# ddlee-cn/LeRF-PyTorch

Measured on AMD Instinct MI355X. Metric: Mpix/s LeRF-G x2 SR (2K->4K), higher is better.
Workload: dtype i32+f32 (u8 io); 1 GPU; LeRF-G LUT x2 SR, 1920x1080->3840x2160 RGB uint8, S=2, max_sigma=10 (BASELINE configs[1]); input=noise, mode=frames, parallelism=independent frames per GPU, no data-path collective, ranks_reported_by_rccl=1, channels=3, library=lerf-pytorch_amd/liblerf_hip.so

## Files before the change

### lerf-pytorch_amd/csrc/lerf_fused_impl.h

```cpp
#include <string.h>
#include <atomic>
#include <type_traits>

#include "lerf_kernels.h"
#include "lerf_stage3.h"
#include "lerf_warp_px.h"

namespace lerf {
namespace LERF_FUSED_NS {

#ifndef LERF_FUSED_NT
#define LERF_FUSED_NT 1024
#endif
constexpr int NT = LERF_FUSED_NT;
constexpr int NW = NT / 64;
constexpr int CH = LERF_FUSED_CH;
static_assert(CH == 1 || CH == 3 || CH == 4, "192 pixel-channels per tile row");
#ifndef LERF_FUSED_TH
#define LERF_FUSED_TH 64
#endif
constexpr int TH = LERF_FUSED_TH, TW = 192 / CH;
constexpr int R1 = 3, R2 = 3;
constexpr int MAXM = 4;
constexpr int LUT_PAD = 83584;
// ... 201 lines not shown
    __device__ __forceinline__ uint32_t ld32(int n) const { return n >= 3 ? lds_ld32<ALL>(a(n)) : lds_ld32<0>(a(n)); }
    __device__ __forceinline__ int ldi8(int n) const { return n >= 3 ? lds_ldi8<ALL>(a(n)) : lds_ldi8<0>(a(n)); }
};

template <int STRIDE_SCALE>
__device__ __forceinline__ Walk<STRIDE_SCALE> simplex_walk(unsigned ka, int basea, uint32_t rb, uint32_t rc, uint32_t rd,
                                                           unsigned sb, unsigned sc, unsigned sd) {
    Walk<STRIDE_SCALE> W;
    const unsigned kb = key_of(rb, sb), kc = key_of(rc, sc), kd = key_of(rd, sd);
    const unsigned t = __umul24(__umul24(msb_of(rb), (unsigned)kL) + msb_of(rc), (unsigned)kL) + msb_of(rd);
    W.i0 = basea + (int)(t * STRIDE_SCALE);
    const unsigned m = umax3(ka, kb, kc), e = umed3(ka, kb, kc), n = umin3(ka, kb, kc);
    const unsigned s0 = m > kd ? m : kd;
    const unsigned s1 = umed3(m, e, kd);
    const unsigned s2 = umed3(e, n, kd);
    const unsigned s3 = n < kd ? n : kd;
    W.i1 = W.i0 + (int)(s0 & 0xFFFFu);
    W.i2 = W.i1 + (int)(s1 & 0xFFFFu);
    W.i3m = W.i0 - (int)(s3 & 0xFFFFu);
    W.f0 = s0 >> 16; W.f1 = s1 >> 16; W.f2 = s2 >> 16; W.f3 = s3 >> 16;
    W.k0 = s0; W.k1 = s1; W.k2 = s2; W.k3 = s3;
    return W;
}

template <int BYTES>
struct Stage16 {
    static constexpr int n = (BYTES + 15) >> 4;
    static constexpr int FULL = n / NT;
    static constexpr int TAIL = n - FULL * NT;
    uint4 r[FULL];
    uint4 rt;
    __device__ __forceinline__ void load(const uint8_t* __restrict__ src, int tid) {
        const uint4* s = reinterpret_cast<const uint4*>(src);
#pragma unroll
        for (int i = 0; i < FULL; ++i) r[i] = s[tid + i * NT];
        rt = make_uint4(0, 0, 0, 0);
        if (TAIL > 0 && tid < TAIL) rt = s[tid + FULL * NT];
    }
    __device__ __forceinline__ void store(uint8_t* dst, int tid) const {
        uint4* d = reinterpret_cast<uint4*>(dst);
#pragma unroll
        for (int i = 0; i < FULL; ++i) d[tid + i * NT] = r[i];
        if (TAIL > 0 && tid < TAIL) d[tid + FULL * NT] = rt;
    }
};

template <int BYTES>
__device__ __forceinline__ void copy16(uint8_t* dst, const uint8_t* __restrict__ src, int tid) {
    Stage16<BYTES> st;
    st.load(src, tid);
    st.store(dst, tid);
}

template <int SP>
__host__ __device__ constexpr int min_tile_offset(char mode, int rot0, int nrot, int rstep) {
    int m = 0;
    for (int i = 0; i < nrot; ++i) {
        const Off3 o = tile_offsets<SP>(mode, rot0 + i * rstep);
        for (int k = 0; k < 3; ++k) m = o.o[k] < m ? o.o[k] : m;
    }
    return m;
}
template <int SP>
__host__ __device__ constexpr int block3_offset(int i) {
    const int dy = i < 3 ? -1 : (i < 5 ? 0 : 1);
    const int dx = i < 3 ? i - 1 : (i < 5 ? (i == 3 ? -1 : 1) : i - 6);
    return dy * SP + dx * CH;
}
template <int SP>
__host__ __device__ constexpr int block3_index(int off) {
    for (int i = 0; i < 8; ++i)
        if (block3_offset<SP>(i) == off) return i;
    return 0;
}
template <int SP, char MODE, int ROT, int MINO>
__device__ __forceinline__ void load_rotation(uint32_t base, uint32_t& rb, uint32_t& rc, uint32_t& rd) {
    constexpr Off3 o = tile_offsets<SP>(MODE, ROT);
    rb = lds_pixel_hi_off<o.o[0] - MINO>(base);
    rc = lds_pixel_hi_off<o.o[1] - MINO>(base);
    rd = lds_pixel_hi_off<o.o[2] - MINO>(base);
}

template <int NROT>
__device__ __forceinline__ int byte_walks(uint32_t lut_a, uint32_t ra, const uint32_t (&rb)[4], const uint32_t (&rc)[4],
                                          const uint32_t (&rd)[4]) {
    const unsigned sa = kStrideA, sb = kStrideB, sc = kStrideC, sd = kStrideD;
    const unsigned ka = key_of(ra, sa);
    const int basea = (int)(__umul24(msb_of(ra), kStrideA) + lut_a);
    Walk<1> W[NROT];
    int e[NROT][5];
#ifndef LERF_S1_SPLIT
#define LERF_S1_SPLIT 1
#endif
#if LERF_S1_SPLIT > 0
#pragma unroll
    for (int h = 0; h < NROT; h += LERF_S1_SPLIT) {
#pragma unroll
        for (int i = h; i < h + LERF_S1_SPLIT; ++i) W[i] = simplex_walk<1>(ka, basea, rb[i], rc[i], rd[i], sb, sc, sd);
#pragma unroll
        for (int i = h; i < h + LERF_S1_SPLIT; ++i)
#pragma unroll
            for (int n = 0; n < 5; ++n) e[i][n] = W[i].ldi8(n);
        __builtin_amdgcn_sched_barrier(0);
    }
#else
#pragma unroll
    for (int i = 0; i < NROT; ++i) W[i] = simplex_walk<1>(ka, basea, rb[i], rc[i], rd[i], sb, sc, sd);
#pragma unroll
    for (int i = 0; i < NROT; ++i)
#pragma unroll
        for (int n = 0; n < 5; ++n) e[i][n] = W[i].ldi8(n);
    __builtin_amdgcn_sched_barrier(0);
#endif
    int acc = 0, sum0 = 0;
#pragma unroll
    for (int i = 0; i < NROT; ++i) {
        sum0 += e[i][0];
#ifndef LERF_S1_MUL24
        acc = mad_i16_keyhi(e[i][1] - e[i][0], W[i].k0, acc);
        acc = mad_i16_keyhi(e[i][2] - e[i][1], W[i].k1, acc);
        acc = mad_i16_keyhi(e[i][3] - e[i][2], W[i].k2, acc);
        acc = mad_i16_keyhi(e[i][4] - e[i][3], W[i].k3, acc);
#else
        acc += __mul24((int)W[i].f0, e[i][1] - e[i][0]);
        acc += __mul24((int)W[i].f1, e[i][2] - e[i][1]);
        acc += __mul24((int)W[i].f2, e[i][3] - e[i][2]);
        acc += __mul24((int)W[i].f3, e[i][4] - e[i][3]);
#endif
    }
    return acc + kQ * sum0;
}


template <int SP, char MODE, int ROT0, int NROT, int RSTEP>
__device__ __forceinline__ int byte_lookups(uint32_t lut_a, uint32_t center) {
    static_assert(NROT == 2 || NROT == 4, "rotation pairs or all four");
    constexpr int MINO = min_tile_offset<SP>(MODE, ROT0, NROT, RSTEP);
    const uint32_t base = center + (uint32_t)MINO;
    uint32_t ra = lds_pixel_hi_off<-MINO>(base);
    uint32_t rb[4], rc[4], rd[4];
    if constexpr (MODE == 's' && NROT == 4 && ROT0 == 0 && RSTEP == 1) {
        uint32_t nb[8];
        nb[0] = lds_pixel_hi_off<block3_offset<SP>(0) - MINO>(base); nb[1] = lds_pixel_hi_off<block3_offset<SP>(1) - MINO>(base);
        nb[2] = lds_pixel_hi_off<block3_offset<SP>(2) - MINO>(base); nb[3] = lds_pixel_hi_off<block3_offset<SP>(3) - MINO>(base);
        nb[4] = lds_pixel_hi_off<block3_offset<SP>(4) - MINO>(base); nb[5] = lds_pixel_hi_off<block3_offset<SP>(5) - MINO>(base);
        nb[6] = lds_pixel_hi_off<block3_offset<SP>(6) - MINO>(base); nb[7] = lds_pixel_hi_off<block3_offset<SP>(7) - MINO>(base);
        asm volatile("s_waitcnt lgkmcnt(0)"
                     : "+v"(ra), "+v"(nb[0]), "+v"(nb[1]), "+v"(nb[2]), "+v"(nb[3]), "+v"(nb[4]), "+v"(nb[5]), "+v"(nb[6]), "+v"(nb[7]));
#pragma unroll
        for (int r = 0; r < 4; ++r) {
            const Off3 o = tile_offsets<SP>('s', r);
            rb[r] = nb[block3_index<SP>(o.o[0])];
            rc[r] = nb[block3_index<SP>(o.o[1])];
            rd[r] = nb[block3_index<SP>(o.o[2])];
        }
    } else {
    load_rotation<SP, MODE, ROT0, MINO>(base, rb[0], rc[0], rd[0]);
    load_rotation<SP, MODE, ROT0 + RSTEP, MINO>(base, rb[1], rc[1], rd[1]);
    if constexpr (NROT == 4) {
        load_rotation<SP, MODE, ROT0 + 2 * RSTEP, MINO>(base, rb[2], rc[2], rd[2]);
        load_rotation<SP, MODE, ROT0 + 3 * RSTEP, MINO>(base, rb[3], rc[3], rd[3]);
        asm volatile("s_waitcnt lgkmcnt(0)"
                     : "+v"(ra), "+v"(rb[0]), "+v"(rc[0]), "+v"(rd[0]), "+v"(rb[1]), "+v"(rc[1]), "+v"(rd[1]), "+v"(rb[2]),
                       "+v"(rc[2]), "+v"(rd[2]), "+v"(rb[3]), "+v"(rc[3]), "+v"(rd[3]));
    } else {
        asm volatile("s_waitcnt lgkmcnt(0)" : "+v"(ra), "+v"(rb[0]), "+v"(rc[0]), "+v"(rd[0]), "+v"(rb[1]), "+v"(rc[1]), "+v"(rd[1]));
    }
    }
    return byte_walks<NROT>(lut_a, ra, rb, rc, rd);
}

template <int NROT>
__device__ __forceinline__ int byte_lookups_rt(uint32_t lut_a, uint32_t center, const int* __restrict__ o) {
    static_assert(NROT == 2 || NROT == 4, "rotation pairs or all four");
    uint32_t ra = lds_pixel_hi(center);
    uint32_t rb[4], rc[4], rd[4];
#pragma unroll
    for (int i = 0; i < NROT; ++i) {
        rb[i] = lds_pixel_hi(center + (uint32_t)o[3 * i]);
        rc[i] = lds_pixel_hi(center + (uint32_t)o[3 * i + 1]);
        rd[i] = lds_pixel_hi(center + (uint32_t)o[3 * i + 2]);
    }
    if constexpr (NROT == 4)
        asm volatile("s_waitcnt lgkmcnt(0)"
                     : "+v"(ra), "+v"(rb[0]), "+v"(rc[0]), "+v"(rd[0]), "+v"(rb[1]), "+v"(rc[1]), "+v"(rd[1]), "+v"(rb[2]),
                       "+v"(rc[2]), "+v"(rd[2]), "+v"(rb[3]), "+v"(rc[3]), "+v"(rd[3]));
    else
        asm volatile("s_waitcnt lgkmcnt(0)" : "+v"(ra), "+v"(rb[0]), "+v"(rc[0]), "+v"(rd[0]), "+v"(rb[1]), "+v"(rc[1]), "+v"(rd[1]));
    return byte_walks<NROT>(lut_a, ra, rb, rc, rd);
}

template <int DPc, int SP>
__device__ __forceinline__ int center_addr(int p, int y0g, int x0g, int sy0g, int sx0g, int H, int W, bool* inside) {
    int ry = p / DPc;
    int r3 = p - ry * DPc;
    if (H < 0) {
        if (inside) *inside = true;
        return (ry + (y0g - sy0g)) * SP + r3 + (x0g - sx0g) * CH;
    }
    int rx = r3 / CH;
    int c = r3 - rx * CH;
    int gy = y0g + ry, gx = x0g + rx;
    int cy = clampi(gy, 0, H - 1), cx = clampi(gx, 0, W - 1);
    if (inside) *inside = (cy == gy) && (cx == gx);
    return (cy - sy0g) * SP + (cx - sx0g) * CH + c;
}

template <int NDST, int DPc, int SP, char MODE, int ROT0, int NROT, int RSTEP, int PHASE>
__device__ __forceinline__ void byte_position(uint32_t lut_a, uint32_t center, int16_t* acc16, uint8_t* dst8, int p, int div, int bias) {
    int v = byte_lookups<SP, MODE, ROT0, NROT, RSTEP>(lut_a, center);
    if (PHASE != 0) v += (int)acc16[p];
    if (PHASE == 2)
        dst8[p] = (uint8_t)rne_div_clip255_fast(v + bias * div, div);
// ... 8 lines not shown
    if (H < 0) {
        constexpr int FULL = NDST / NT, TAIL = NDST - FULL * NT;
        const uint32_t org = src_a + (uint32_t)((y0g - sy0g) * SP + (x0g - sx0g) * CH);
#pragma unroll 1
        for (int k = 0; k < FULL; ++k) {
            const int p = tid + k * NT;
            const int ry = p / DPc;
            byte_position<NDST, DPc, SP, MODE, ROT0, NROT, RSTEP, PHASE>(lut_a, org + (uint32_t)(ry * (SP - DPc) + p), acc16, dst8, p, div, bias);
        }
        if (TAIL > 0 && tid < TAIL) {
            const int p = tid + FULL * NT;
            const int ry = p / DPc;
            byte_position<NDST, DPc, SP, MODE, ROT0, NROT, RSTEP, PHASE>(lut_a, org + (uint32_t)(ry * (SP - DPc) + p), acc16, dst8, p, div, bias);
        }
        return;
    }
    for (int p = tid; p < NDST; p += NT) {
        bool in = true;
        int a = center_addr<DPc, SP>(p, y0g, x0g, sy0g, sx0g, H, W, SKIP_OUTSIDE ? &in : nullptr);
        if (SKIP_OUTSIDE && !in) continue;
        byte_position<NDST, DPc, SP, MODE, ROT0, NROT, RSTEP, PHASE>(lut_a, src_a + (uint32_t)a, acc16, dst8, p, div, bias);
    }
}

struct DyDx { int dy[3], dx[3]; };
__host__ __device__ constexpr DyDx pattern_dydx(char mode, int rot) {
    int dy[4] = {0, 0, 0, 0}, dx[4] = {0, 0, 0, 0};
    switch (mode) {
        case 's': dy[1] = 0; dx[1] = 1; dy[2] = 1; dx[2] = 0; dy[3] = 1; dx[3] = 1; break;
        case 'd': dy[1] = 0; dx[1] = 2; dy[2] = 2; dx[2] = 0; dy[3] = 2; dx[3] = 2; break;
        case 'y': dy[1] = 1; dx[1] = 1; dy[2] = 1; dx[2] = 2; dy[3] = 2; dx[3] = 1; break;
        case 'c': dy[1] = 0; dx[1] = 1; dy[2] = 0; dx[2] = 2; dy[3] = 0; dx[3] = 3; break;
        default:  dy[1] = 1; dx[1] = 1; dy[2] = 2; dx[2] = 2; dy[3] = 3; dx[3] = 3; break;
    }
    DyDx r{};
    for (int k = 1; k < 4; ++k) {
        int y = dy[k], x = dx[k];
        for (int i = 0; i < (rot & 3); ++i) { int t = y; y = x; x = -t; }
        r.dy[k - 1] = y;
        r.dx[k - 1] = x;
    }
    return r;
}
template <int IMM>
__device__ __forceinline__ uint32_t gl_pixel_hi(uint32_t voff, uint64_t rowbase) {
    uint32_t r;
    asm volatile("global_load_ubyte_d16_hi %0, %1, %2 offset:%3" : "=v"(r) : "v"(voff), "s"(rowbase), "n"(IMM));
    return r;
}
struct PixSet { uint32_t a, b[4], c[4], d[4]; };
template <char MODE, int ROT0, int NROT, int RSTEP>
__device__ __forceinline__ void pix_issue(PixSet& P, uint32_t voff, const uint64_t (&rows)[7]) {
    P.a = gl_pixel_hi<0>(voff, rows[3]);
#define LERF_PX(I, K) gl_pixel_hi<pattern_dydx(MODE, ROT0 + (I) * RSTEP).dx[K] * CH>(voff, rows[pattern_dydx(MODE, ROT0 + (I) * RSTEP).dy[K] + 3])
    if constexpr (MODE == 's' && NROT == 4 && ROT0 == 0 && RSTEP == 1) {
        P.b[0] = LERF_PX(0, 0); P.b[1] = LERF_PX(1, 0); P.b[2] = LERF_PX(2, 0); P.b[3] = LERF_PX(3, 0);
        P.d[0] = LERF_PX(0, 2); P.d[1] = LERF_PX(1, 2); P.d[2] = LERF_PX(2, 2); P.d[3] = LERF_PX(3, 2);
    } else {
        P.b[0] = LERF_PX(0, 0); P.c[0] = LERF_PX(0, 1); P.d[0] = LERF_PX(0, 2);
        P.b[1] = LERF_PX(1, 0); P.c[1] = LERF_PX(1, 1); P.d[1] = LERF_PX(1, 2);
        if constexpr (NROT == 4) {
            P.b[2] = LERF_PX(2, 0); P.c[2] = LERF_PX(2, 1); P.d[2] = LERF_PX(2, 2);
            P.b[3] = LERF_PX(3, 0); P.c[3] = LERF_PX(3, 1); P.d[3] = LERF_PX(3, 2);
        }
    }
#undef LERF_PX
}
template <char MODE, int ROT0, int NROT, int RSTEP>
__device__ __forceinline__ void pix_ready(PixSet& P) {
    if constexpr (MODE == 's' && NROT == 4 && ROT0 == 0 && RSTEP == 1) {
        asm volatile("s_waitcnt vmcnt(0)" : "+v"(P.a), "+v"(P.b[0]), "+v"(P.b[1]), "+v"(P.b[2]), "+v"(P.b[3]), "+v"(P.d[0]), "+v"(P.d[1]),
                     "+v"(P.d[2]), "+v"(P.d[3]));
        static_assert(pattern_dydx('s', 0).dy[1] == pattern_dydx('s', 1).dy[0] && pattern_dydx('s', 0).dx[1] == pattern_dydx('s', 1).dx[0],
                      "pixel c of rotation r = pixel b of rotation r + 1");
        P.c[0] = P.b[1]; P.c[1] = P.b[2]; P.c[2] = P.b[3]; P.c[3] = P.b[0];
    } else if constexpr (NROT == 4) {
        asm volatile("s_waitcnt vmcnt(0)"
                     : "+v"(P.a), "+v"(P.b[0]), "+v"(P.c[0]), "+v"(P.d[0]), "+v"(P.b[1]), "+v"(P.c[1]), "+v"(P.d[1]), "+v"(P.b[2]),
                       "+v"(P.c[2]), "+v"(P.d[2]), "+v"(P.b[3]), "+v"(P.c[3]), "+v"(P.d[3]));
    } else {
        asm volatile("s_waitcnt vmcnt(0)" : "+v"(P.a), "+v"(P.b[0]), "+v"(P.c[0]), "+v"(P.d[0]), "+v"(P.b[1]), "+v"(P.c[1]), "+v"(P.d[1]));
    }
}
template <int NDST, int DPc, char MODE, int ROT0, int NROT, int RSTEP, int PHASE>
__device__ __forceinline__ void byte_phase_vmem(const int8_t* lut, const uint8_t* __restrict__ origin, int pitch, int16_t* acc16,
                                                uint8_t* dst8, int div, int bias, int tid) {
    constexpr int ROUNDS = (NDST + NT - 1) / NT, PAIRS = (ROUNDS + 1) / 2;
    const uint32_t lut_a = lds_addr(lut);
    uint64_t rows[7];
#pragma unroll
    for (int dy = -3; dy <= 3; ++dy) rows[dy + 3] = (uint64_t)reinterpret_cast<uintptr_t>(origin + (int64_t)dy * pitch);
    auto voff_of = [&](int p) {
        p = p < NDST ? p : NDST - 1;
        const int ry = p / DPc;
        return (uint32_t)(ry * pitch + (p - ry * DPc));
    };
    auto finish = [&](const PixSet& X, int p) {
        if (NDST % NT != 0 && p >= NDST) return;
        int v = byte_walks<NROT>(lut_a, X.a, X.b, X.c, X.d);
        if (PHASE != 0) v += (int)acc16[p];
        if (PHASE == 2)
            dst8[p] = (uint8_t)rne_div_clip255_fast(v + bias * div, div);
        else
            acc16[p] = (int16_t)v;
    };
    PixSet A, B;
    pix_issue<MODE, ROT0, NROT, RSTEP>(A, voff_of(tid), rows);
#pragma unroll 1
    for (int k = 0; k < PAIRS; ++k) {
        const int p = tid + 2 * k * NT;
        pix_ready<MODE, ROT0, NROT, RSTEP>(A);
        pix_issue<MODE, ROT0, NROT, RSTEP>(B, voff_of(p + NT), rows);
        finish(A, p);
        pix_ready<MODE, ROT0, NROT, RSTEP>(B);
        if (k + 1 < PAIRS) pix_issue<MODE, ROT0, NROT, RSTEP>(A, voff_of(p + 2 * NT), rows);
        if (2 * k + 1 < ROUNDS) finish(B, p + NT);
    }
}

__device__ __forceinline__ uint32_t gl_pixel_hi_rt(uint32_t voff, uint64_t origin) {
    uint32_t r;
    asm volatile("global_load_ubyte_d16_hi %0, %1, %2" : "=v"(r) : "v"(voff), "s"(origin));
    return r;
}
template <int NDST, int DPc, int NROT>
__device__ __forceinline__ void byte_phase_vmem_rt(const int8_t* lut, const uint8_t* __restrict__ origin, int pitch, int16_t* acc16,
                                                   uint8_t* dst8, int div, int bias, int tid, const int* __restrict__ dyx, bool first,
                                                   bool last) {
    constexpr int ROUNDS = (NDST + NT - 1) / NT, PAIRS = (ROUNDS + 1) / 2;
    const uint32_t lut_a = lds_addr(lut);
    const int reach = 3 * pitch + 3 * CH;
    const uint64_t org = (uint64_t)reinterpret_cast<uintptr_t>(origin - reach);
    int off[NROT * 3];
#pragma unroll
    for (int i = 0; i < NROT * 3; ++i) off[i] = (dyx[i] >> 16) * pitch + (int)(int16_t)(dyx[i] & 0xFFFF) * CH;
    auto voff_of = [&](int p) {
        p = p < NDST ? p : NDST - 1;
        const int ry = p / DPc;
        return (uint32_t)(ry * pitch + (p - ry * DPc) + reach);
    };
    auto issue = [&](PixSet& X, uint32_t voff) {
        X.a = gl_pixel_hi_rt(voff, org);
#pragma unroll
        for (int i = 0; i < NROT; ++i) {
            X.b[i] = gl_pixel_hi_rt(voff + (uint32_t)off[3 * i], org);
            X.c[i] = gl_pixel_hi_rt(voff + (uint32_t)off[3 * i + 1], org);
            X.d[i] = gl_pixel_hi_rt(voff + (uint32_t)off[3 * i + 2], org);
        }
    };
    auto ready = [&](PixSet& X) {
        if constexpr (NROT == 4)
            asm volatile("s_waitcnt vmcnt(0)"
                         : "+v"(X.a), "+v"(X.b[0]), "+v"(X.c[0]), "+v"(X.d[0]), "+v"(X.b[1]), "+v"(X.c[1]), "+v"(X.d[1]), "+v"(X.b[2]),
                           "+v"(X.c[2]), "+v"(X.d[2]), "+v"(X.b[3]), "+v"(X.c[3]), "+v"(X.d[3]));
        else
            asm volatile("s_waitcnt vmcnt(0)" : "+v"(X.a), "+v"(X.b[0]), "+v"(X.c[0]), "+v"(X.d[0]), "+v"(X.b[1]), "+v"(X.c[1]), "+v"(X.d[1]));
    };
    auto finish = [&](const PixSet& X, int p) {
        if (NDST % NT != 0 && p >= NDST) return;
        int v = byte_walks<NROT>(lut_a, X.a, X.b, X.c, X.d);
        if (!first) v += (int)acc16[p];
        if (last)
            dst8[p] = (uint8_t)rne_div_clip255_fast(v + bias * div, div);
        else
            acc16[p] = (int16_t)v;
    };
    PixSet A, B;
    issue(A, voff_of(tid));
#pragma unroll 1
    for (int k = 0; k < PAIRS; ++k) {
        const int p = tid + 2 * k * NT;
        ready(A);
        issue(B, voff_of(p + NT));
        finish(A, p);
        ready(B);
        if (k + 1 < PAIRS) issue(A, voff_of(p + 2 * NT));
        if (2 * k + 1 < ROUNDS) finish(B, p + NT);
    }
}

template <int NROT>
__device__ __forceinline__ void byte_position_rt(uint32_t lut_a, uint32_t center, int16_t* acc16, uint8_t* dst8, int p, int div,
                                                 int bias, const int* __restrict__ o, bool first, bool last) {
    int v = byte_lookups_rt<NROT>(lut_a, center, o);
    if (!first) v += (int)acc16[p];
    if (last)
        dst8[p] = (uint8_t)rne_div_clip255_fast(v + bias * div, div);
    else
        acc16[p] = (int16_t)v;
}
template <int NDST, int DPc, int SP, int NROT, bool SKIP_OUTSIDE = false>
__device__ __forceinline__ void byte_phase_rt(const int8_t* lut, const uint8_t* src, int16_t* acc16, uint8_t* dst8, int y0g, int x0g,
                                              int sy0g, int sx0g, int H, int W, int div, int bias, int tid,
                                              const int* __restrict__ o, bool first, bool last) {
    const uint32_t lut_a = lds_addr(lut), src_a = lds_addr(src);
    if (H < 0) {
        const uint32_t org = src_a + (uint32_t)((y0g - sy0g) * SP + (x0g - sx0g) * CH);
#pragma unroll 1
        for (int p = tid; p < NDST; p += NT) {
            const int ry = p / DPc;
// ... 282 lines not shown
        const bool dwords = interior && (D::FP & 3) == 0 && ((W * CH) & 3) == 0 && (reinterpret_cast<uintptr_t>(F.feat) & 3) == 0 && ((fx0 * CH) & 3) == 0;
        if (dwords) {
            constexpr int RD = D::FP / 4, ND = D::FY * RD, KD = (ND + NT - 1) / NT;
            const uint32_t* src = reinterpret_cast<const uint32_t*>(fsrc + ((int64_t)fy0 * W + fx0) * CH);
            const int rowdw = (W * CH) >> 2;
            uint32_t v[KD];
#pragma unroll
            for (int k = 0; k < KD; ++k) {
                const int p = min(tid + k * NT, ND - 1);
                const int ry = p / RD;
                v[k] = __builtin_nontemporal_load(&src[(int64_t)ry * rowdw + (p - ry * RD)]);
            }
            if (D::GEO_EARLY && !EMIT && !WARP) geo_search();
#pragma unroll
            for (int k = 0; k < KD; ++k) {
                const int p = tid + k * NT;
                if (p < ND) reinterpret_cast<uint32_t*>(Bt)[p] = v[k];
            }
        } else {
            constexpr int KI = (D::NF + NT - 1) / NT;
            uint8_t v[KI];
#pragma unroll
            for (int k = 0; k < KI; ++k) {
                const int p = min(tid + k * NT, D::NF - 1);
                const int ry = p / D::FP;
                const int r3 = p - ry * D::FP;
                const int rx = r3 / CH;
                const int gy = clampi(fy0 + ry, 0, H - 1), gx = clampi(fx0 + rx, 0, W - 1);
                v[k] = fsrc[((int64_t)gy * W + gx) * CH + (r3 - rx * CH)];
            }
            if (D::GEO_EARLY && !EMIT && !WARP) geo_search();
#pragma unroll
            for (int k = 0; k < KI; ++k) {
                const int p = tid + k * NT;
                if (p < D::NF) Bt[p] = v[k];
            }
        }
        __syncthreads();
        if (D::GEO_EARLY && !EMIT && !WARP) geo_stage();
        LERF_STAMP(6);
    }

    uint32_t* Dt = reinterpret_cast<uint32_t*>(smem + D::OFF_D);

    auto outside_pixel = [&](int gy, int gx, int c) -> uint32_t {
        if (P.pad_mode == LERF_PAD_CONSTANT) return 0u;
        bool zy, zx;
        const int sy = pad_index(gy, H, P.pad_mode, &zy), sx = pad_index(gx, W, P.pad_mode, &zx);
        const int ry = sy - fy0, rx = sx - fx0;
        if (ry >= 0 && ry < D::FY && rx >= 0 && rx < D::FX) return (uint32_t)Bt[ry * D::FP + rx * CH + c];
        if (FROM_FEAT) return (uint32_t)F.feat[((int64_t)sy * W + sx) * CH + c];
        return 0u;
    };

    if (KIND == LERF_KIND_LINEAR) {
        int8_t* lut = reinterpret_cast<int8_t*>(smem + D::OFF_LUT);
        int16_t* acc = reinterpret_cast<int16_t*>(smem + D::OFF_ACC);
        uint8_t* hq8 = smem + D::OFF_C;
        const uint8_t* s2 = P.pack + (size_t)(GEN ? P.n1 : 3) * LUT_PAD;
        const int div2 = kQ * 12;
        constexpr int L2N = (LERF_LUT_ENTRIES + 15) / 16, L2TAIL = L2N - 5 * NT;
        static_assert(L2TAIL > 0 && L2TAIL <= NT, "byte LUT = 5 full uint4 rounds + a tail");
        uint4 m0, m1, m2, m3, m4, m5 = make_uint4(0, 0, 0, 0);
#define LERF_L2_LOAD(IDX)                                                                          \
        do {                                                                                       \
            const uint4* s_ = reinterpret_cast<const uint4*>(s2 + (IDX) * LUT_PAD);                \
            m0 = s_[tid]; m1 = s_[tid + NT]; m2 = s_[tid + 2 * NT]; m3 = s_[tid + 3 * NT]; m4 = s_[tid + 4 * NT]; \
            if (tid < L2TAIL) m5 = s_[tid + 5 * NT];                                               \
        } while (0)
#define LERF_L2_STORE()                                                                            \
        do {                                                                                       \
            uint4* d_ = reinterpret_cast<uint4*>(smem + D::OFF_LUT);                               \
            d_[tid] = m0; d_[tid + NT] = m1; d_[tid + 2 * NT] = m2; d_[tid + 3 * NT] = m3; d_[tid + 4 * NT] = m4; \
            if (tid < L2TAIL) d_[tid + 5 * NT] = m5;                                               \
        } while (0)
#ifndef LERF_S1_LDS_PIXELS
        const bool vm2 = FROM_FEAT && !GEN && interior;
#else
        const bool vm2 = false;
#endif
        const uint8_t* forg = FROM_FEAT ? F.feat + ((int64_t)hy0 * W + hx0) * CH : nullptr;
        const int fpitch = W * CH;
#define LERF_L2(NEXT, MODE, PAR, PH)                                                                       \
        if ((NEXT) < 6) LERF_L2_LOAD(NEXT);                                                                \
        if (vm2) byte_phase_vmem<D::NH, D::HP, MODE, PAR, 2, 2, PH>(lut, forg, fpitch, acc, hq8, div2, 127, tid); \
        else byte_phase<D::NH, D::HP, D::FP, MODE, PAR, 2, 2, PH>(lut, Bt, acc, hq8, hy0, hx0, fy0, fx0, Hc, Wc, div2, 127, tid); \
        __syncthreads();                                                                                   \
        if ((NEXT) < 6) {                                                                                  \
            LERF_L2_STORE();                                                                               \
            __syncthreads();                                                                               \
        }
        copy16<LERF_LUT_ENTRIES>(smem + D::OFF_LUT, s2 + 0 * LUT_PAD, tid);
        __syncthreads();
        if constexpr (GEN) {
            const int nl = 2 * P.n2, dv = kQ * 4 * P.n2;
#pragma unroll 1
            for (int l = 0; l < nl; ++l) {
                const bool more = l + 1 < nl;
                if (more) LERF_L2_LOAD(l + 1);
                if (FROM_FEAT && interior)
                    byte_phase_vmem_rt<D::NH, D::HP, 2>(lut, forg, fpitch, acc, hq8, dv, 127, tid, P.s2dyx[l], l == 0, !more);
                else
                byte_phase_rt<D::NH, D::HP, D::FP, 2>(lut, Bt, acc, hq8, hy0, hx0, fy0, fx0, Hc, Wc, dv, 127, tid, P.s2off[l], l == 0, !more);
                __syncthreads();
                if (more) {
                    LERF_L2_STORE();
                    __syncthreads();
                }
            }
        } else {
        LERF_L2(1, 's', 0, 0)
        LERF_L2(2, 's', 1, 1)
        LERF_L2(3, 'c', 0, 1)
        LERF_L2(4, 'c', 1, 1)
        LERF_L2(5, 't', 0, 1)
        LERF_L2(6, 't', 1, 2)
        }
#undef LERF_L2
#undef LERF_L2_LOAD
#undef LERF_L2_STORE
        uint32_t tmp[(D::NH + NT - 1) / NT];
#pragma unroll
        for (int k = 0; k < (D::NH + NT - 1) / NT; ++k) {
            int p = k * NT + tid;
            tmp[k] = 0;
            if (p < D::NH) {
                bool inside;
                int a = center_addr<D::HP, D::FP>(p, hy0, hx0, fy0, fx0, Hc, Wc, &inside);
                uint32_t px = 0u;
                if (inside) px = (uint32_t)Bt[a];
                else if (P.pad_mode != LERF_PAD_CONSTANT) {
                    const int ry = p / D::HP, r3 = p - ry * D::HP, rx = r3 / CH;
                    px = outside_pixel(hy0 + ry, hx0 + rx, r3 - rx * CH);
                }
                tmp[k] = (uint32_t)hq8[p] | (px << 24);
            }
        }
        __syncthreads();
#pragma unroll
        for (int k = 0; k < (D::NH + NT - 1) / NT; ++k) {
            int p = k * NT + tid;
            if (p < D::NH) Dt[p] = tmp[k];
        }
    } else {
        constexpr int MAXR = D::MAXR;
        uint16_t* lst = reinterpret_cast<uint16_t*>(smem + D::OFF_LST);
        int* tab = reinterpret_cast<int*>(smem + D::OFF_TAB);
        for (int i = tid; i < MAXR * NT / 2; i += NT) reinterpret_cast<uint32_t*>(lst)[i] = 0xFFFFFFFFu;
        constexpr int KH = (D::NH + NT - 1) / NT;
        static_assert(KH <= 15 && NBIN <= 4 && NW == 16, "nibble counts, one byte field per bin, one lane per (wave, bin)");
        uint32_t qlo = 0, qhi = 0;
        uint32_t xa, xb;
        {
            uint32_t hist = 0;
#pragma unroll
            for (int k = 0; k < KH; ++k) {
                const int p = tid * KH + k;
                uint32_t q = 15;
                if (p < D::NH) {
                    bool in = true;
                    const int a = center_addr<D::HP, D::FP>(p, hy0, hx0, fy0, fx0, Hc, Wc, &in);
#ifndef LERF_FULL_RING
                    if (D::HR > 0) {
                        const int ry = p / D::HP, r3 = p - ry * D::HP;
                        if (ry == D::HY - 1 || r3 >= (D::HX - 1) * CH) in = false;
                    }
#endif
                    if (in) q = bin_of_level((uint32_t)Bt[a] >> 4);
                }
// ... 946 lines not shown
#pragma unroll
                            for (int b = 0; b < S; ++b) dd[a * S + b] = Dt[(lr + b) * D::HP + (lc + a) * CH + c];
                        outt[il * D::OUT_PITCH + ophase + xc] = (uint8_t)s3::resolve_u8<KIND == LERF_KIND_GAUSS, S>(dd, dx64, dy64, P.max_sigma);
                    }
                    __syncthreads();
                }
            }
            flush_blocks();
        } else if (F.dis_r64 != nullptr) {
            asm volatile("s_waitcnt vmcnt(0)" ::: "memory");
            __syncthreads();
            const int nq = min(*tq_count, P.tq_cap);
            for (int i = tid; i < nq; i += NT) {
                const uint32_t e = tq[i];
                const int il = (int)(e >> 16), xc = (int)(e & 0xFFFFu);
                const int jl = xc / CH;
                const int c = xc - jl * CH;
                const int lr = g_lr[il], lc = g_lc[jl];
                uint32_t dd[SS];
                double dx64[S], dy64[S];
#pragma unroll
                for (int b = 0; b < S; ++b) dx64[b] = F.dis_r64[(int64_t)(i0 + il) * S + b];
#pragma unroll
                for (int a = 0; a < S; ++a) dy64[a] = F.dis_c64[(int64_t)(j0 + jl) * S + a];
#pragma unroll
                for (int a = 0; a < S; ++a)
#pragma unroll
                    for (int b = 0; b < S; ++b) dd[a * S + b] = Dt[(lr + b) * D::HP + (lc + a) * CH + c];
                seg0[il * rowpitch + xc] = (uint8_t)s3::resolve_u8<KIND == LERF_KIND_GAUSS, S>(dd, dx64, dy64, P.max_sigma);
            }
        }
    }
#ifdef LERF_STAMPS
    __syncthreads();
    LERF_STAMP(12);
    LERF_STAMP_RT(14);
#endif
}

constexpr int up16c(int x) { return (x + 15) / 16 * 16; }
struct DimsA {
    static constexpr int FY = TH, FX = TW, FP = FX * CH, NF = FY * FP;
    static constexpr int IY = FY + 2 * R1, IX = FX + 2 * R1, IPB = IX * CH, IP = (IPB + 3 + 3) / 4 * 4, NI = IY * IP;
    static constexpr int OFF_LUT = 0;
    static constexpr int OFF_C = LUT_PAD;
    static constexpr int OFF_ACC = OFF_C + up16c(NI);
    static constexpr int OFF_F = OFF_ACC + up16c(NF * 2);
    static constexpr int LDS_BYTES = OFF_F + up16c(NF);
};

template <bool GEN = false>
__global__ void __launch_bounds__(NT)
s1_kernel(Params P, std::conditional_t<GEN, RaggedTable, NoTable> T) {
    using D = DimsA;
    extern __shared__ __attribute__((aligned(16))) uint8_t smem[];
    const int tid = threadIdx.x;
    int bid = xcd_order((int)blockIdx.x, (int)gridDim.x);
    const FrameView F = frame_view<GEN>(P, T, bid);
    const int tyi = bid / F.tiles_x, txi = bid - tyi * F.tiles_x;
    const int fy0 = P.ty_org + tyi * TH, fx0 = P.tx_org + txi * TW;
    const int iy0 = fy0 - R1, ix0 = fx0 - R1;
    const int H = F.H, W = F.W;
    const uint8_t* __restrict__ img = F.img;
    const bool interior = iy0 >= 0 && ix0 >= 0 && iy0 + D::IY <= H && ix0 + D::IX <= W;
    const int Hc = interior ? -1 : H, Wc = W;
    uint8_t* Ft = smem + D::OFF_F;
    LERF_STAMP(0);

#ifndef LERF_S1_LDS_PIXELS
    const bool vmem_pixels = !GEN && interior && !P.host_input;
#else
    const bool vmem_pixels = false;
#endif
    if (vmem_pixels) {
        int8_t* lut = reinterpret_cast<int8_t*>(smem + D::OFF_LUT);
        int16_t* acc = reinterpret_cast<int16_t*>(smem + D::OFF_ACC);
        const int div1 = kQ * 3;
        const uint8_t* org = img + ((int64_t)fy0 * W + fx0) * CH;
        const int pitch = W * CH;
        constexpr int L1N = (LERF_LUT_ENTRIES + 15) / 16, L1TAIL = L1N - 5 * NT;
        uint4 n0, n1, n2, n3, n4, n5 = make_uint4(0, 0, 0, 0);
        copy16<LERF_LUT_ENTRIES>(smem + D::OFF_LUT, P.pack + 0 * LUT_PAD, tid);
        __syncthreads();
        LERF_S1_LOAD(P.pack + 1 * LUT_PAD);
        byte_phase_vmem<D::NF, D::FP, 's', 0, 4, 1, 0>(lut, org, pitch, acc, Ft, div1, 0, tid);
        __syncthreads();
        LERF_S1_STORE();
        __syncthreads();
        LERF_S1_LOAD(P.pack + 2 * LUT_PAD);
        byte_phase_vmem<D::NF, D::FP, 'c', 0, 4, 1, 1>(lut, org, pitch, acc, Ft, div1, 0, tid);
        __syncthreads();
        LERF_S1_STORE();
        __syncthreads();
        byte_phase_vmem<D::NF, D::FP, 't', 0, 4, 1, 2>(lut, org, pitch, acc, Ft, div1, 0, tid);
        __syncthreads();
    } else {
    const int cphase = load_input_tile<D::IY, D::IPB, D::IP>(smem + D::OFF_C, img, H, W, iy0, ix0, interior, tid, []() {});
    {
        const uint8_t* Ct = smem + D::OFF_C + cphase;
        int8_t* lut = reinterpret_cast<int8_t*>(smem + D::OFF_LUT);
        int16_t* acc = reinterpret_cast<int16_t*>(smem + D::OFF_ACC);
        const int div1 = kQ * 3;
        constexpr int L1N = (LERF_LUT_ENTRIES + 15) / 16, L1TAIL = L1N - 5 * NT;
        uint4 n0, n1, n2, n3, n4, n5 = make_uint4(0, 0, 0, 0);
        copy16<LERF_LUT_ENTRIES>(smem + D::OFF_LUT, P.pack + 0 * LUT_PAD, tid);
        __syncthreads();
        if constexpr (GEN) {
            const int dv = kQ * P.n1;
            const bool vmg = interior && !P.host_input;
            const uint8_t* vorg = img + ((int64_t)fy0 * W + fx0) * CH;
#pragma unroll 1
            for (int m = 0; m < P.n1; ++m) {
                const bool more = m + 1 < P.n1;
                if (more) LERF_S1_LOAD(P.pack + (size_t)(m + 1) * LUT_PAD);
                if (vmg) byte_phase_vmem_rt<D::NF, D::FP, 4>(lut, vorg, W * CH, acc, Ft, dv, 0, tid, P.s1dyx[m], m == 0, !more);
                else
                byte_phase_rt<D::NF, D::FP, D::IP, 4, true>(lut, Ct, acc, Ft, fy0, fx0, iy0, ix0, Hc, Wc, dv, 0, tid, P.s1off[m], m == 0, !more);
                __syncthreads();
                if (more) {
                    LERF_S1_STORE();
                    __syncthreads();
                }
            }
        } else {
        LERF_S1_LOAD(P.pack + 1 * LUT_PAD);
        byte_phase<D::NF, D::FP, D::IP, 's', 0, 4, 1, 0, true>(lut, Ct, acc, Ft, fy0, fx0, iy0, ix0, Hc, Wc, div1, 0, tid);
        __syncthreads();
        LERF_S1_STORE();
        __syncthreads();
        LERF_S1_LOAD(P.pack + 2 * LUT_PAD);
        byte_phase<D::NF, D::FP, D::IP, 'c', 0, 4, 1, 1, true>(lut, Ct, acc, Ft, fy0, fx0, iy0, ix0, Hc, Wc, div1, 0, tid);
        __syncthreads();
        LERF_S1_STORE();
        __syncthreads();
        byte_phase<D::NF, D::FP, D::IP, 't', 0, 4, 1, 2, true>(lut, Ct, acc, Ft, fy0, fx0, iy0, ix0, Hc, Wc, div1, 0, tid);
        __syncthreads();
        }
    }
    }
    LERF_STAMP(1);
    uint8_t* __restrict__ fdst = F.feat;
    const int rows = min(TH, H - fy0), cols3 = min(TW, W - fx0) * CH;
    const bool dwords = cols3 == D::FP && ((W * CH) & 3) == 0 && (reinterpret_cast<uintptr_t>(F.feat) & 3) == 0;
    if (dwords) {
        constexpr int RD = D::FP / 4;
        uint32_t* dst = reinterpret_cast<uint32_t*>(fdst + ((int64_t)fy0 * W + fx0) * CH);
        const int rowdw = (W * CH) >> 2;
        for (int i = tid; i < rows * RD; i += NT) {
            const int r = i / RD;
            __builtin_nontemporal_store(reinterpret_cast<const uint32_t*>(Ft)[i], &dst[(int64_t)r * rowdw + (i - r * RD)]);
        }
    } else {
        for (int i = tid; i < rows * cols3; i += NT) {
            const int r = i / cols3, c3 = i - r * cols3;
            fdst[((int64_t)(fy0 + r) * W + fx0) * CH + c3] = Ft[r * D::FP + c3];
        }
    }
#ifdef LERF_STAMPS
    __syncthreads();
    LERF_STAMP(2);
#endif
}

#undef LERF_S1_LOAD
#undef LERF_S1_STORE
#undef LERF_ADDTID
#undef LERF_ADDTID4
#undef LERF_SET_M0


template <auto KERN>
static int ensure_lds(int bytes) {
    static std::atomic<uint64_t> done{0};
    int dev = 0;
    if (hipGetDevice(&dev) != hipSuccess) return LERF_ELAUNCH;
    const uint64_t bit = 1ull << (dev & 63);
    if (done.load(std::memory_order_relaxed) & bit) return LERF_OK;
// ... 176 lines not shown
```

Measured before the change: 28990 Mpix/s.

## Software-pipeline LUT walks across pixel rounds and defer next-LUT prefetch to tail

Splits byte_walks into an issue step (simplex walk plus LDS LUT byte loads) and a consume step, so the vmem pixel phase can start the next pixel's LUT reads (half or all rotations ahead) while the current pixel is still being accumulated. The loop is restructured into paired rounds with an explicit tail. The global load of the next LUT plane is passed in as a prefetch callback and issued near the end of the phase instead of before it, which shortens the time its registers stay live. This raises register pressure through the pending walk state and adds complexity to the tail handling.

New measurement: 29160 Mpix/s (median of 6 runs). No clear change (+0.6%).

```diff
diff --git a/lerf-pytorch_amd/csrc/lerf_fused_impl.h b/lerf-pytorch_amd/csrc/lerf_fused_impl.h
--- a/lerf-pytorch_amd/csrc/lerf_fused_impl.h
+++ b/lerf-pytorch_amd/csrc/lerf_fused_impl.h
@@ -307,53 +307,73 @@
 }
 
 template <int NROT>
-__device__ __forceinline__ int byte_walks(uint32_t lut_a, uint32_t ra, const uint32_t (&rb)[4], const uint32_t (&rc)[4],
-                                          const uint32_t (&rd)[4]) {
+struct WalksPending {
+    int e[NROT][5];
+    unsigned k[NROT][4];
+};
+#ifndef LERF_S1_SPLIT
+#define LERF_S1_SPLIT 1
+#endif
+template <int NROT, int LO, int HI>
+__device__ __forceinline__ void byte_walks_issue(WalksPending<NROT>& Q, uint32_t lut_a, uint32_t ra, const uint32_t (&rb)[4],
+                                                 const uint32_t (&rc)[4], const uint32_t (&rd)[4]) {
+    static_assert(0 <= LO && LO < HI && HI <= NROT, "a range of rotations");
     const unsigned sa = kStrideA, sb = kStrideB, sc = kStrideC, sd = kStrideD;
     const unsigned ka = key_of(ra, sa);
     const int basea = (int)(__umul24(msb_of(ra), kStrideA) + lut_a);
     Walk<1> W[NROT];
-    int e[NROT][5];
-#ifndef LERF_S1_SPLIT
-#define LERF_S1_SPLIT 1
-#endif
 #if LERF_S1_SPLIT > 0
-#pragma unroll
-    for (int h = 0; h < NROT; h += LERF_S1_SPLIT) {
+    static_assert((HI - LO) % LERF_S1_SPLIT == 0, "whole groups of walks");
+#pragma unroll
+    for (int h = LO; h < HI; h += LERF_S1_SPLIT) {
 #pragma unroll
         for (int i = h; i < h + LERF_S1_SPLIT; ++i) W[i] = simplex_walk<1>(ka, basea, rb[i], rc[i], rd[i], sb, sc, sd);
 #pragma unroll
         for (int i = h; i < h + LERF_S1_SPLIT; ++i)
 #pragma unroll
-            for (int n = 0; n < 5; ++n) e[i][n] = W[i].ldi8(n);
+            for (int n = 0; n < 5; ++n) Q.e[i][n] = W[i].ldi8(n);
         __builtin_amdgcn_sched_barrier(0);
     }
 #else
 #pragma unroll
-    for (int i = 0; i < NROT; ++i) W[i] = simplex_walk<1>(ka, basea, rb[i], rc[i], rd[i], sb, sc, sd);
-#pragma unroll
-    for (int i = 0; i < NROT; ++i)
-#pragma unroll
-        for (int n = 0; n < 5; ++n) e[i][n] = W[i].ldi8(n);
+    for (int i = LO; i < HI; ++i) W[i] = simplex_walk<1>(ka, basea, rb[i], rc[i], rd[i], sb, sc, sd);
+#pragma unroll
+    for (int i = LO; i < HI; ++i)
+#pragma unroll
+        for (int n = 0; n < 5; ++n) Q.e[i][n] = W[i].ldi8(n);
     __builtin_amdgcn_sched_barrier(0);
 #endif
+#pragma unroll
+    for (int i = LO; i < HI; ++i) {
+        Q.k[i][0] = W[i].k0; Q.k[i][1] = W[i].k1; Q.k[i][2] = W[i].k2; Q.k[i][3] = W[i].k3;
+    }
+}
+template <int NROT>
+__device__ __forceinline__ int byte_walks_consume(const WalksPending<NROT>& Q) {
     int acc = 0, sum0 = 0;
 #pragma unroll
     for (int i = 0; i < NROT; ++i) {
-        sum0 += e[i][0];
+        sum0 += Q.e[i][0];
 #ifndef LERF_S1_MUL24
-        acc = mad_i16_keyhi(e[i][1] - e[i][0], W[i].k0, acc);
-        acc = mad_i16_keyhi(e[i][2] - e[i][1], W[i].k1, acc);
-        acc = mad_i16_keyhi(e[i][3] - e[i][2], W[i].k2, acc);
-        acc = mad_i16_keyhi(e[i][4] - e[i][3], W[i].k3, acc);
+        acc = mad_i16_keyhi(Q.e[i][1] - Q.e[i][0], Q.k[i][0], acc);
+        acc = mad_i16_keyhi(Q.e[i][2] - Q.e[i][1], Q.k[i][1], acc);
+        acc = mad_i16_keyhi(Q.e[i][3] - Q.e[i][2], Q.k[i][2], acc);
+        acc = mad_i16_keyhi(Q.e[i][4] - Q.e[i][3], Q.k[i][3], acc);
 #else
-        acc += __mul24((int)W[i].f0, e[i][1] - e[i][0]);
-        acc += __mul24((int)W[i].f1, e[i][2] - e[i][1]);
-        acc += __mul24((int)W[i].f2, e[i][3] - e[i][2]);
-        acc += __mul24((int)W[i].f3, e[i][4] - e[i][3]);
+        acc += __mul24((int)(Q.k[i][0] >> 16), Q.e[i][1] - Q.e[i][0]);
+        acc += __mul24((int)(Q.k[i][1] >> 16), Q.e[i][2] - Q.e[i][1]);
+        acc += __mul24((int)(Q.k[i][2] >> 16), Q.e[i][3] - Q.e[i][2]);
+        acc += __mul24((int)(Q.k[i][3] >> 16), Q.e[i][4] - Q.e[i][3]);
 #endif
     }
     return acc + kQ * sum0;
+}
+template <int NROT>
+__device__ __forceinline__ int byte_walks(uint32_t lut_a, uint32_t ra, const uint32_t (&rb)[4], const uint32_t (&rc)[4],
+                                          const uint32_t (&rd)[4]) {
+    WalksPending<NROT> Q;
+    byte_walks_issue<NROT, 0, NROT>(Q, lut_a, ra, rb, rc, rd);
+    return byte_walks_consume<NROT>(Q);
 }
 
 
@@ -528,9 +548,19 @@
         asm volatile("s_waitcnt vmcnt(0)" : "+v"(P.a), "+v"(P.b[0]), "+v"(P.c[0]), "+v"(P.d[0]), "+v"(P.b[1]), "+v"(P.c[1]), "+v"(P.d[1]));
     }
 }
-template <int NDST, int DPc, char MODE, int ROT0, int NROT, int RSTEP, int PHASE>
+#ifndef LERF_S1_PIPE
+#define LERF_S1_PIPE 1
+#endif
+#ifndef LERF_S1_PIXLATE
+#define LERF_S1_PIXLATE 0
+#endif
+#ifndef LERF_S1_LUTTAIL
+#define LERF_S1_LUTTAIL (LERF_S1_PIPE > 0)
+#endif
+static_assert(LERF_S1_PIPE >= 0 && LERF_S1_PIPE <= 2, "LERF_S1_PIPE: 0 off, 1 half a position ahead, 2 a whole position");
+template <int NDST, int DPc, char MODE, int ROT0, int NROT, int RSTEP, int PHASE, class Prefetch>
 __device__ __forceinline__ void byte_phase_vmem(const int8_t* lut, const uint8_t* __restrict__ origin, int pitch, int16_t* acc16,
-                                                uint8_t* dst8, int div, int bias, int tid) {
+                                                uint8_t* dst8, int div, int bias, int tid, Prefetch&& prefetch) {
     constexpr int ROUNDS = (NDST + NT - 1) / NT, PAIRS = (ROUNDS + 1) / 2;
     const uint32_t lut_a = lds_addr(lut);
     uint64_t rows[7];
@@ -541,6 +571,7 @@
         const int ry = p / DPc;
         return (uint32_t)(ry * pitch + (p - ry * DPc));
     };
+#if LERF_S1_PIPE == 0
     auto finish = [&](const PixSet& X, int p) {
         if (NDST % NT != 0 && p >= NDST) return;
         int v = byte_walks<NROT>(lut_a, X.a, X.b, X.c, X.d);
@@ -550,6 +581,7 @@
         else
             acc16[p] = (int16_t)v;
     };
+    prefetch();
     PixSet A, B;
     pix_issue<MODE, ROT0, NROT, RSTEP>(A, voff_of(tid), rows);
 #pragma unroll 1
@@ -562,6 +594,57 @@
         if (k + 1 < PAIRS) pix_issue<MODE, ROT0, NROT, RSTEP>(A, voff_of(p + 2 * NT), rows);
         if (2 * k + 1 < ROUNDS) finish(B, p + NT);
     }
+#else
+    constexpr int AHEAD = LERF_S1_PIPE == 1 ? NROT / 2 : NROT;
+    auto live = [&](int p) { return NDST % NT == 0 || p < NDST; };
+    auto round = [&](PixSet& Xc, WalksPending<NROT>& Qc, PixSet& Xn, WalksPending<NROT>& Qn, int p, bool more, bool pix)
+                     __attribute__((always_inline)) {
+        int prev = 0;
+        if (PHASE != 0 && live(p)) prev = (int)acc16[p];
+        if constexpr (AHEAD < NROT)
+            if (live(p)) byte_walks_issue<NROT, AHEAD, NROT>(Qc, lut_a, Xc.a, Xc.b, Xc.c, Xc.d);
+        if (more) pix_ready<MODE, ROT0, NROT, RSTEP>(Xn);
+        if (!LERF_S1_PIXLATE && pix) pix_issue<MODE, ROT0, NROT, RSTEP>(Xc, voff_of(p + 2 * NT), rows);
+        if (more && live(p + NT)) byte_walks_issue<NROT, 0, AHEAD>(Qn, lut_a, Xn.a, Xn.b, Xn.c, Xn.d);
+        if (live(p)) {
+            const int v = byte_walks_consume<NROT>(Qc) + prev;
+            if (PHASE == 2)
+                dst8[p] = (uint8_t)rne_div_clip255_fast(v + bias * div, div);
+            else
+                acc16[p] = (int16_t)v;
+        }
+        if (LERF_S1_PIXLATE && pix) pix_issue<MODE, ROT0, NROT, RSTEP>(Xc, voff_of(p + 2 * NT), rows);
+    };
+    if (!LERF_S1_LUTTAIL) prefetch();
+    PixSet A, B;
+    WalksPending<NROT> QA, QB;
+    pix_issue<MODE, ROT0, NROT, RSTEP>(A, voff_of(tid), rows);
+    pix_ready<MODE, ROT0, NROT, RSTEP>(A);
+    if (ROUNDS > 1) pix_issue<MODE, ROT0, NROT, RSTEP>(B, voff_of(tid + NT), rows);
+    if (live(tid)) byte_walks_issue<NROT, 0, AHEAD>(QA, lut_a, A.a, A.b, A.c, A.d);
+    constexpr int TAIL = ROUNDS % 2 == 0 ? 2 : (ROUNDS < 3 ? ROUNDS : 3), R0 = ROUNDS - TAIL;
+    constexpr int LUTAT = TAIL - (LERF_S1_LUTTAIL == 1 && TAIL >= 2 ? 2 : 1);
+    static_assert(R0 % 2 == 0, "whole pairs in the loop");
+#pragma unroll 1
+    for (int k = 0; k < R0 / 2; ++k) {
+        const int p = tid + 2 * k * NT;
+        round(A, QA, B, QB, p, true, true);
+        round(B, QB, A, QA, p + NT, true, true);
+    }
+    {
+        const int p = tid + R0 * NT;
+        if (LERF_S1_LUTTAIL && LUTAT == 0) prefetch();
+        round(A, QA, B, QB, p, 1 < TAIL, 2 < TAIL);
+        if constexpr (TAIL > 1) {
+            if (LERF_S1_LUTTAIL && LUTAT == 1) prefetch();
+            round(B, QB, A, QA, p + NT, 2 < TAIL, false);
+        }
+        if constexpr (TAIL > 2) {
+            if (LERF_S1_LUTTAIL && LUTAT == 2) prefetch();
+            round(A, QA, B, QB, p + 2 * NT, false, false);
+        }
+    }
+#endif
 }
 
 __device__ __forceinline__ uint32_t gl_pixel_hi_rt(uint32_t voff, uint64_t origin) {
@@ -1010,9 +1093,12 @@
         const uint8_t* forg = FROM_FEAT ? F.feat + ((int64_t)hy0 * W + hx0) * CH : nullptr;
         const int fpitch = W * CH;
 #define LERF_L2(NEXT, MODE, PAR, PH)                                                                       \
-        if ((NEXT) < 6) LERF_L2_LOAD(NEXT);                                                                \
-        if (vm2) byte_phase_vmem<D::NH, D::HP, MODE, PAR, 2, 2, PH>(lut, forg, fpitch, acc, hq8, div2, 127, tid); \
-        else byte_phase<D::NH, D::HP, D::FP, MODE, PAR, 2, 2, PH>(lut, Bt, acc, hq8, hy0, hx0, fy0, fx0, Hc, Wc, div2, 127, tid); \
+        if (vm2) byte_phase_vmem<D::NH, D::HP, MODE, PAR, 2, 2, PH>(lut, forg, fpitch, acc, hq8, div2, 127, tid, \
+                                                                    [&]() { if ((NEXT) < 6) LERF_L2_LOAD(NEXT); }); \
+        else {                                                                                             \
+            if ((NEXT) < 6) LERF_L2_LOAD(NEXT);                                                            \
+            byte_phase<D::NH, D::HP, D::FP, MODE, PAR, 2, 2, PH>(lut, Bt, acc, hq8, hy0, hx0, fy0, fx0, Hc, Wc, div2, 127, tid); \
+        }                                                                                                  \
         __syncthreads();                                                                                   \
         if ((NEXT) < 6) {                                                                                  \
             LERF_L2_STORE();                                                                               \
@@ -2125,17 +2211,15 @@
         uint4 n0, n1, n2, n3, n4, n5 = make_uint4(0, 0, 0, 0);
         copy16<LERF_LUT_ENTRIES>(smem + D::OFF_LUT, P.pack + 0 * LUT_PAD, tid);
         __syncthreads();
-        LERF_S1_LOAD(P.pack + 1 * LUT_PAD);
-        byte_phase_vmem<D::NF, D::FP, 's', 0, 4, 1, 0>(lut, org, pitch, acc, Ft, div1, 0, tid);
+        byte_phase_vmem<D::NF, D::FP, 's', 0, 4, 1, 0>(lut, org, pitch, acc, Ft, div1, 0, tid, [&]() { LERF_S1_LOAD(P.pack + 1 * LUT_PAD); });
         __syncthreads();
         LERF_S1_STORE();
         __syncthreads();
-        LERF_S1_LOAD(P.pack + 2 * LUT_PAD);
-        byte_phase_vmem<D::NF, D::FP, 'c', 0, 4, 1, 1>(lut, org, pitch, acc, Ft, div1, 0, tid);
+        byte_phase_vmem<D::NF, D::FP, 'c', 0, 4, 1, 1>(lut, org, pitch, acc, Ft, div1, 0, tid, [&]() { LERF_S1_LOAD(P.pack + 2 * LUT_PAD); });
         __syncthreads();
         LERF_S1_STORE();
         __syncthreads();
-        byte_phase_vmem<D::NF, D::FP, 't', 0, 4, 1, 2>(lut, org, pitch, acc, Ft, div1, 0, tid);
+        byte_phase_vmem<D::NF, D::FP, 't', 0, 4, 1, 2>(lut, org, pitch, acc, Ft, div1, 0, tid, []() {});
         __syncthreads();
     } else {
     const int cphase = load_input_tile<D::IY, D::IPB, D::IP>(smem + D::OFF_C, img, H, W, iy0, ix0, interior, tid, []() {});
```
